# somepago/DCR

Measured on AMD Instinct MI355X. Metric: sd21_256px_finetune_imgs_per_sec, higher is better.
Workload: dtype bf16; 1 GPU; model=sd2.1-unet-865M-random-init, global_batch=16, resolution=256, seq_len=77, parallelism=dp1, optimizer=fused_adamw

## Files before the change

### dcr_amd/__main__.py

```python
import hashlib
import platform

import torch

import dcr_amd
from dcr_amd import ops


def main():
    print(f"dcr_amd {dcr_amd.__version__}")
    print(f"torch {torch.__version__} (hip {torch.version.hip})")
    print(f"python {platform.python_version()} on {platform.machine()}")
    print(f"cuda/hip device available: {torch.cuda.is_available()}")
    m = ops.ext()
    if m is None:
        print("HIP extension: NOT BUILT (run __graft_entry__.build())")
    else:
        kernels = sorted(n for n in dir(m) if not n.startswith("_"))
        from pathlib import Path
        so = Path(ops.__file__).parent / "_dcr_hip.so"
        digest = hashlib.sha256(so.read_bytes()).hexdigest()[:16]
        print(f"HIP extension: {so} (sha256 {digest})")
        print(f"  exported ops ({len(kernels)}): {', '.join(kernels)}")
    if ops.dispatch_counts:
        print(f"dispatch counts: {dict(ops.dispatch_counts)}")
    import os
    gates = ["DCR_NATIVE_CONV", "DCR_NATIVE_CONV_BWD", "DCR_NATIVE_GEMM",
             "DCR_ATTN_V4", "DCR_ATTN_BWD_V4", "DCR_HIPGRAPH",
             "DCR_ATTN_V2", "DCR_DEV_ADAMW", "DCR_PROFILE",
             "DCR_AMD_ALLOW_FALLBACK"]
    active = {g: os.environ[g] for g in gates if g in os.environ}
    desc = active if active else "defaults (native conv on; round-2 drafts off)"
    print(f"env gates: {desc}")


if __name__ == "__main__":
    main()
```

### dcr_amd/ops/hip/bindings.cpp

```cpp

#include <torch/extension.h>
#include <ATen/cuda/CUDAContext.h>

#include "dcr_launchers.h"

using namespace dcr;

namespace {

DType dtype_of(const at::Tensor& t) {
  switch (t.scalar_type()) {
    case at::kFloat: return DT_F32;
    case at::kHalf: return DT_F16;
    case at::kBFloat16: return DT_BF16;
    default: TORCH_CHECK(false, "dcr_hip: unsupported dtype ", t.scalar_type());
  }
}

hipStream_t cur_stream() {
  return at::cuda::getCurrentCUDAStream().stream();
}

at::Tensor as_f32(const at::Tensor& t) {
  return t.scalar_type() == at::kFloat ? t.contiguous()
// ... 449 lines not shown

std::vector<at::Tensor> attn_fwd_gen_lse(at::Tensor q, at::Tensor k,
                                         at::Tensor v, double scale,
                                         bool causal) {
  at::Tensor lse;
  auto o = attn_fwd_gen_impl(q, k, v, scale, causal, &lse);
  return {o, lse};
}

std::vector<at::Tensor> attn_bwd_gen(at::Tensor q, at::Tensor k, at::Tensor v,
                                     at::Tensor o, at::Tensor dO,
                                     at::Tensor lse, double scale,
                                     bool causal) {
  int64_t B, H, Lq, Lk, D;
  attn_gen_dims(q, k, v, B, H, Lq, Lk, D);
  TORCH_CHECK(k.sizes() == v.sizes(), "attn_bwd_gen: k/v shape mismatch");
  TORCH_CHECK(o.sizes() == q.sizes() && dO.sizes() == q.sizes(),
              "attn_bwd_gen: o/dO must have q's shape");
  TORCH_CHECK(o.is_cuda() && dO.is_cuda() && lse.is_cuda() &&
              o.scalar_type() == at::kBFloat16 &&
              dO.scalar_type() == at::kBFloat16 &&
              o.is_contiguous() && dO.is_contiguous(),
              "attn_bwd_gen: o/dO must be contiguous bf16 CUDA tensors");
  TORCH_CHECK(lse.scalar_type() == at::kFloat && lse.is_contiguous() &&
              lse.dim() == 2 && lse.size(0) == B * H && lse.size(1) == Lq,
              "attn_bwd_gen: lse must be contiguous fp32 [B*H, Lq]");
  auto dQ = at::empty_like(q);
  auto dK = at::empty_like(k);
  auto dV = at::empty_like(v);
  auto delta = at::empty({B * H, Lq}, q.options().dtype(at::kFloat));
  attn_bwd_gen_launch(q.data_ptr(), k.data_ptr(), v.data_ptr(), o.data_ptr(),
                      dO.data_ptr(), lse.data_ptr<float>(),
                      delta.data_ptr<float>(), dQ.data_ptr(), dK.data_ptr(),
                      dV.data_ptr(), (int)(B * H), (int)Lq, (int)Lk, (int)H,
                      (int)D, (float)scale, causal, cur_stream());
  return {dQ, dK, dV};
}

std::vector<at::Tensor> attn_fwd_v4(at::Tensor q, at::Tensor k, at::Tensor v,
                                    double scale, bool causal) {
  TORCH_CHECK(q.is_cuda() && q.scalar_type() == at::kBFloat16,
              "attn: bf16 CUDA only");
  TORCH_CHECK(q.is_contiguous() && k.is_contiguous() && v.is_contiguous());
  int64_t B, H, Lq, Lk;
  attn_dims(q, k, B, H, Lq, Lk);
  auto o = at::empty_like(q);
  auto lse = at::empty({B * H, Lq}, q.options().dtype(at::kFloat));
  attn_fwd_v4_launch(q.data_ptr(), k.data_ptr(), v.data_ptr(), o.data_ptr(),
                     lse.data_ptr<float>(), (int)(B * H), (int)Lq, (int)Lk,
                     (int)H, (float)scale, causal, cur_stream());
  return {o, lse};
}

std::vector<at::Tensor> attn_fwd_v3(at::Tensor q, at::Tensor k, at::Tensor v,
                                    double scale, bool causal) {
  TORCH_CHECK(q.is_cuda() && q.scalar_type() == at::kBFloat16,
              "attn: bf16 CUDA only");
  TORCH_CHECK(q.is_contiguous() && k.is_contiguous() && v.is_contiguous());
  int64_t B, H, Lq, Lk;
  attn_dims(q, k, B, H, Lq, Lk);
  auto o = at::empty_like(q);
  auto lse = at::empty({B * H, Lq}, q.options().dtype(at::kFloat));
  attn_fwd_v3_launch(q.data_ptr(), k.data_ptr(), v.data_ptr(), o.data_ptr(),
                     lse.data_ptr<float>(), (int)(B * H), (int)Lq, (int)Lk,
                     (int)H, (float)scale, causal, cur_stream());
  return {o, lse};
}

std::vector<at::Tensor> attn_fwd_v2(at::Tensor q, at::Tensor k, at::Tensor v,
                                    double scale, bool causal) {
  TORCH_CHECK(q.is_cuda() && q.scalar_type() == at::kBFloat16,
              "attn: bf16 CUDA only");
  TORCH_CHECK(q.is_contiguous() && k.is_contiguous() && v.is_contiguous());
  int64_t B, H, Lq, Lk;
  attn_dims(q, k, B, H, Lq, Lk);
  auto o = at::empty_like(q);
  auto lse = at::empty({B * H, Lq}, q.options().dtype(at::kFloat));
  attn_fwd_v2_launch(q.data_ptr(), k.data_ptr(), v.data_ptr(), o.data_ptr(),
                     lse.data_ptr<float>(), (int)(B * H), (int)Lq, (int)Lk,
                     (int)H, (float)scale, causal, cur_stream());
  return {o, lse};
}

std::vector<at::Tensor> attn_bwd(at::Tensor q, at::Tensor k, at::Tensor v,
                                 at::Tensor o, at::Tensor dO, at::Tensor lse,
                                 double scale, bool causal) {
  int64_t B, H, Lq, Lk;
  attn_dims(q, k, B, H, Lq, Lk);
  auto dQ = at::empty_like(q);
  auto dK = at::empty_like(k);
  auto dV = at::empty_like(v);
  auto delta = at::empty({B * H, Lq}, q.options().dtype(at::kFloat));
  attn_bwd_launch(q.data_ptr(), k.data_ptr(), v.data_ptr(), o.data_ptr(),
                  dO.contiguous().data_ptr(), lse.data_ptr<float>(),
                  delta.data_ptr<float>(), dQ.data_ptr(), dK.data_ptr(),
                  dV.data_ptr(), (int)(B * H), (int)Lq, (int)Lk, (int)H,
                  (float)scale, causal, cur_stream());
  return {dQ, dK, dV};
}

std::vector<at::Tensor> attn_bwd_v4(at::Tensor q, at::Tensor k, at::Tensor v,
                                 at::Tensor o, at::Tensor dO, at::Tensor lse,
                                 double scale, bool causal) {
  int64_t B, H, Lq, Lk;
  attn_dims(q, k, B, H, Lq, Lk);
  auto dQ = at::empty_like(q);
  auto dK = at::empty_like(k);
  auto dV = at::empty_like(v);
  auto delta = at::empty({B * H, Lq}, q.options().dtype(at::kFloat));
  attn_bwd_v4_launch(q.data_ptr(), k.data_ptr(), v.data_ptr(), o.data_ptr(),
                  dO.contiguous().data_ptr(), lse.data_ptr<float>(),
                  delta.data_ptr<float>(), dQ.data_ptr(), dK.data_ptr(),
                  dV.data_ptr(), (int)(B * H), (int)Lq, (int)Lk, (int)H,
                  (float)scale, causal, cur_stream());
  return {dQ, dK, dV};
}


at::Tensor mfma_probe(at::Tensor A, at::Tensor B) {
  TORCH_CHECK(A.is_cuda() && A.scalar_type() == at::kBFloat16);
  TORCH_CHECK(A.sizes() == at::IntArrayRef({16, 32}) &&
              B.sizes() == at::IntArrayRef({32, 16}));
  auto C = at::zeros({16, 16}, A.options().dtype(at::kFloat));
  mfma_probe_launch(A.contiguous().data_ptr(), B.contiguous().data_ptr(),
                    C.data_ptr<float>(), cur_stream());
  return C;
}

static const void* conv_bias_ptr(const c10::optional<at::Tensor>& bias,
                                 at::Tensor& keep, bool& is_bf16) {
  is_bf16 = false;
  if (!bias.has_value()) return nullptr;
  if (bias->scalar_type() == at::kBFloat16) {
    is_bf16 = true;
    keep = bias->contiguous();
  } else {
    keep = as_f32(*bias);
  }
  return keep.data_ptr();
}

at::Tensor conv2d_nhwc_fwd(at::Tensor x, at::Tensor w,
                           c10::optional<at::Tensor> bias, int64_t stride,
                           int64_t pad) {
  TORCH_CHECK(x.is_cuda() && x.scalar_type() == at::kBFloat16);
  TORCH_CHECK(x.is_contiguous(at::MemoryFormat::ChannelsLast) &&
              w.is_contiguous(at::MemoryFormat::ChannelsLast),
              "conv_nhwc: channels_last only");
  const int64_t Nb = x.size(0), C = x.size(1), Hin = x.size(2), Win = x.size(3);
  const int64_t K = w.size(0), R = w.size(2), S = w.size(3);
  TORCH_CHECK(w.size(1) == C && C % 32 == 0 && K % 64 == 0);
  TORCH_CHECK((R == 3 && S == 3) || (R == 1 && S == 1));
  const int64_t P = (Hin + 2 * pad - R) / stride + 1;
  const int64_t Q = (Win + 2 * pad - S) / stride + 1;
  auto y = at::empty({Nb, K, P, Q},
                     x.options().memory_format(at::MemoryFormat::ChannelsLast));
  at::Tensor bf;
  bool b_bf16 = false;
  const void* bp = conv_bias_ptr(bias, bf, b_bf16);
  conv_nhwc_fwd_launch(x.data_ptr(), w.data_ptr(), bp, b_bf16, y.data_ptr(), (int)Nb,
                       (int)Hin, (int)Win, (int)C, (int)K, (int)P, (int)Q,
                       (int)R, (int)S, (int)stride, (int)pad, cur_stream());
  return y;
}

static at::Tensor conv2d_nhwc_fwd_v2_impl(at::Tensor x, at::Tensor w,
                                          c10::optional<at::Tensor> bias,
                                          int64_t stride, int64_t pad,
                                          c10::optional<at::Tensor> res,
                                          c10::optional<at::Tensor> temb) {
  TORCH_CHECK(x.is_cuda() && x.scalar_type() == at::kBFloat16);
  TORCH_CHECK(x.is_contiguous(at::MemoryFormat::ChannelsLast) &&
              w.is_contiguous(at::MemoryFormat::ChannelsLast));
  const int64_t Nb = x.size(0), C = x.size(1), Hin = x.size(2), Win = x.size(3);
  const int64_t K = w.size(0), R = w.size(2), S = w.size(3);
  TORCH_CHECK(w.size(1) == C && C % 32 == 0 && K % 64 == 0);
  TORCH_CHECK((R == 3 && S == 3) || (R == 1 && S == 1));
  const int64_t P = (Hin + 2 * pad - R) / stride + 1;
  const int64_t Q = (Win + 2 * pad - S) / stride + 1;
  auto y = at::empty({Nb, K, P, Q},
                     x.options().memory_format(at::MemoryFormat::ChannelsLast));
  at::Tensor bf;
  bool b_bf16 = false;
  const void* bp = conv_bias_ptr(bias, bf, b_bf16);
  const int64_t NPQ = Nb * P * Q;
  int64_t blocks = ((NPQ + 127) / 128) * ((K + 127) / 128);
  int64_t nsteps = C * R * S / ((C % 64 == 0) ? 64 : 32);
  int splitz = 1;
  if (blocks < 384) {
    splitz = (int)std::min<int64_t>({(384 + blocks - 1) / blocks, nsteps, 16});
    if (splitz < 1) splitz = 1;
  }
  at::Tensor ws;
  float* wsp = nullptr;
  if (splitz > 1) {
    ws = at::zeros({NPQ * K}, x.options().dtype(at::kFloat));
    wsp = ws.data_ptr<float>();
  }
  const void* rp = nullptr;
  const void* tp = nullptr;
  if (res.has_value()) {
    TORCH_CHECK(res->scalar_type() == at::kBFloat16 &&
                res->is_contiguous(at::MemoryFormat::ChannelsLast) &&
                res->sizes() == y.sizes(), "conv res: NHWC bf16 same shape");
    rp = res->data_ptr();
  }
  if (temb.has_value()) {
    TORCH_CHECK(temb->scalar_type() == at::kBFloat16 &&
                temb->is_contiguous() && temb->dim() == 2 &&
                temb->size(0) == Nb && temb->size(1) == K,
                "conv temb: contiguous bf16 [N, K]");
    tp = temb->data_ptr();
  }
  conv_nhwc_fwd_v2_launch(x.data_ptr(), w.data_ptr(), bp, b_bf16, y.data_ptr(), wsp,
         splitz, rp, tp, (int)Nb, (int)Hin, (int)Win, (int)C, (int)K,
         (int)P, (int)Q, (int)R, (int)S, (int)stride,
         (int)pad, cur_stream());
  return y;
}

at::Tensor conv2d_nhwc_fwd_v2(at::Tensor x, at::Tensor w,
                              c10::optional<at::Tensor> bias, int64_t stride,
                              int64_t pad,
                              c10::optional<at::Tensor> res = c10::nullopt,
                              c10::optional<at::Tensor> temb = c10::nullopt) {
  return conv2d_nhwc_fwd_v2_impl(x, w, bias, stride, pad, res, temb);
}

std::vector<at::Tensor> conv2d_nhwc_bwd(at::Tensor dy, at::Tensor x,
                                        at::Tensor w, int64_t stride,
                                        int64_t pad) {
  TORCH_CHECK(dy.is_cuda() && dy.scalar_type() == at::kBFloat16);
  TORCH_CHECK(dy.is_contiguous(at::MemoryFormat::ChannelsLast) &&
              x.is_contiguous(at::MemoryFormat::ChannelsLast) &&
              w.is_contiguous(at::MemoryFormat::ChannelsLast));
  const int64_t Nb = x.size(0), C = x.size(1), Hin = x.size(2), Win = x.size(3);
  const int64_t K = w.size(0), R = w.size(2), S = w.size(3);
  TORCH_CHECK(C % 64 == 0 && K % 64 == 0);
  const int64_t P = dy.size(2), Q = dy.size(3);
  const int64_t NPQ = Nb * P * Q;
  int splits = (int)std::min<int64_t>(std::max<int64_t>(
      384 / std::max<int64_t>((K / 64) * (R * S * C / 32), 1), 1), 16);
  auto dw_ws = at::zeros({K * R * S * C}, x.options().dtype(at::kFloat));
  auto dW = at::empty_like(w);
  conv_bwd_weight_launch(dy.data_ptr(), x.data_ptr(), dw_ws.data_ptr<float>(),
                         (int)Nb, (int)Hin, (int)Win, (int)C, (int)K, (int)P,
                         (int)Q, (int)R, (int)S, (int)stride, (int)pad,
                         splits, dW.data_ptr(), cur_stream());
  auto dx = at::empty_like(x);
  conv_bwd_data_launch(dy.data_ptr(), w.data_ptr(), dx.data_ptr(), (int)Nb,
                       (int)Hin, (int)Win, (int)C, (int)K, (int)P, (int)Q,
                       (int)R, (int)S, (int)stride, (int)pad, cur_stream());
  auto db = at::zeros({K}, x.options().dtype(at::kFloat));
  conv_bias_grad_launch(dy.data_ptr(), db.data_ptr<float>(), NPQ, (int)K,
                        cur_stream());
  return {dx, dW, db};
}

std::vector<at::Tensor> gemm_bf16(at::Tensor A, at::Tensor B,
                                  c10::optional<at::Tensor> bias,
                                  bool ta, bool tb, bool want_dbias) {
  TORCH_CHECK(A.is_cuda() && A.scalar_type() == at::kBFloat16 &&
              B.scalar_type() == at::kBFloat16, "gemm_bf16: bf16 CUDA only");
  TORCH_CHECK(A.is_contiguous() && B.is_contiguous());
  TORCH_CHECK(A.dim() == 2 && B.dim() == 2);
  const int64_t M = ta ? A.size(1) : A.size(0);
  const int64_t K = ta ? A.size(0) : A.size(1);
  const int64_t N = tb ? B.size(1) : B.size(0);
  TORCH_CHECK((tb ? B.size(0) : B.size(1)) == K, "gemm_bf16: K mismatch");
  TORCH_CHECK(K % 8 == 0, "gemm_bf16: K % 8 != 0");
  auto C = at::empty({M, N}, A.options());
  at::Tensor bf;
  const float* bp = nullptr;
  if (bias.has_value()) {
    bf = bias->to(at::kFloat).contiguous();
    bp = bf.data_ptr<float>();
  }
  const int64_t blocks = ((M + 127) / 128) * ((N + 127) / 128);
  const int64_t nsteps = (K + 63) / 64;
  int splitz = 1;
  if (blocks < 384)
    splitz = (int)std::min<int64_t>({(384 + blocks - 1) / blocks, nsteps, 16});
  if (splitz < 1) splitz = 1;
  at::Tensor ws;
  float* wsp = nullptr;
  if (splitz > 1) {
    ws = at::zeros({M * N}, A.options().dtype(at::kFloat));
    wsp = ws.data_ptr<float>();
  }
  at::Tensor db;
  float* dbp = nullptr;
  if (want_dbias) {
    TORCH_CHECK(ta, "gemm_bf16: dbias fusion needs ta (wgrad layout)");
    db = at::zeros({M}, A.options().dtype(at::kFloat));
    dbp = db.data_ptr<float>();
  }
  gemm_bf16_launch(A.data_ptr(), B.data_ptr(), bp, C.data_ptr(), wsp, dbp,
                   M, N, (int)K, ta ? 1 : 0, tb ? 1 : 0, want_dbias ? 1 : 0,
                   splitz, cur_stream());
  if (want_dbias) return {C, db};
  return {C};
}

PYBIND11_MODULE(TORCH_EXTENSION_NAME, mod) {
  mod.def("gemm_bf16", &gemm_bf16);
  mod.def("conv2d_nhwc_bwd", &conv2d_nhwc_bwd);
  mod.def("conv2d_nhwc_fwd", &conv2d_nhwc_fwd);
  mod.def("conv2d_nhwc_fwd_v2", &conv2d_nhwc_fwd_v2,
          pybind11::arg("x"), pybind11::arg("w"), pybind11::arg("bias"),
          pybind11::arg("stride"), pybind11::arg("pad"),
          pybind11::arg("res") = c10::nullopt,
          pybind11::arg("temb") = c10::nullopt);
  mod.def("attn_fwd", &attn_fwd);
  mod.def("attn_fwd_gen", &attn_fwd_gen);
  mod.def("attn_fwd_gen_lse", &attn_fwd_gen_lse);
  mod.def("attn_bwd_gen", &attn_bwd_gen);
  mod.def("attn_fwd_v2", &attn_fwd_v2);
  mod.def("attn_fwd_v3", &attn_fwd_v3);
  mod.def("attn_fwd_v4", &attn_fwd_v4);
  mod.def("attn_bwd", &attn_bwd);
  mod.def("attn_bwd_v4", &attn_bwd_v4);
  mod.def("mfma_probe", &mfma_probe);
  mod.def("groupnorm_silu_fwd", &groupnorm_silu_fwd);
  mod.def("groupnorm_silu_bwd", &groupnorm_silu_bwd);
  mod.def("groupnorm_silu_nhwc_fwd", &groupnorm_silu_nhwc_fwd);
  mod.def("groupnorm_silu_nhwc_bwd", &groupnorm_silu_nhwc_bwd);
  mod.def("layernorm_fwd", &layernorm_fwd);
  mod.def("layernorm_bwd", &layernorm_bwd, py::arg("dy"), py::arg("x"),
          py::arg("w"), py::arg("mean"), py::arg("rstd"),
          py::arg("blocks") = 0);
  mod.def("colsum", &colsum);
  mod.def("colsum_grouped", &colsum_grouped);
  mod.def("geglu_fwd", &geglu_fwd);
  mod.def("geglu_bwd", &geglu_bwd);
  mod.def("adamw_step", &adamw_step);
  mod.def("adamw_step_bf16", &adamw_step_bf16);
  mod.def("adamw_step_dev", &adamw_step_dev);
  mod.def("adamw8_step", &adamw8_step, py::arg("p"), py::arg("g"),
          py::arg("exp_avg_q"), py::arg("exp_avg_absmax"),
          py::arg("exp_avg_sq_q"), py::arg("exp_avg_sq_absmax"), py::arg("lr"),
          py::arg("beta1"), py::arg("beta2"), py::arg("eps"), py::arg("wd"),
          py::arg("step"));
  mod.def("adamw8_step_bf16", &adamw8_step_bf16, py::arg("p"), py::arg("g"),
          py::arg("master"), py::arg("exp_avg_q"), py::arg("exp_avg_absmax"),
          py::arg("exp_avg_sq_q"), py::arg("exp_avg_sq_absmax"), py::arg("lr"),
          py::arg("beta1"), py::arg("beta2"), py::arg("eps"), py::arg("wd"),
          py::arg("step"));
  mod.def("add_noise", &add_noise);
  mod.def("get_velocity", &get_velocity);
  mod.def("cfg_combine", &cfg_combine);
  mod.def("lincomb", &lincomb);
}
```

### dcr_amd/ops/hip/dcr_launchers.h

```cpp
#pragma once

#include <hip/hip_runtime.h>

namespace dcr {

enum DType { DT_F32 = 0, DT_F16 = 1, DT_BF16 = 2 };

void gn_fwd_launch(DType dt, const void* x, const void* w, const void* b,
                   bool w_f32, void* y, float* mean, float* rstd, int NG,
                   int G, int Cg, int HW, float eps, bool silu, hipStream_t s);
void gn_bwd_launch(DType dt, const void* dy, const void* x, const void* w,
                   const void* b, bool w_f32, const float* mean,
                   const float* rstd, void* dx, float* dw, float* db, int NG,
                   int G, int Cg, int HW, bool silu, hipStream_t s);
void ln_fwd_launch(DType dt, const void* x, const void* w, const void* b,
                   bool w_f32, void* y, float* mean, float* rstd, long M,
                   int N, float eps, hipStream_t s);
void ln_bwd_launch(DType dt, const void* dy, const void* x, const void* w,
                   bool w_f32, const float* mean, const float* rstd, void* dx,
                   float* dw, float* db, long M, int N, hipStream_t s);
int ln_bwd_v2_blocks(long M, int N);
void ln_bwd_v2_launch(DType dt, const void* dy, const void* x, const void* w,
                      bool w_f32, const float* mean, const float* rstd,
                      void* dx, float* slab, void* dwdb, int blocks, long M,
                      int N, hipStream_t s);

int gn_nhwc_chunks(int N, int R);
void gn_nhwc_fwd_launch(DType dt, const void* x, const void* w, const void* b,
                        bool w_f32, void* y, float* ws, float* mean, float* rstd,
                        int N, int R, int C, int G, float eps, bool silu,
                        hipStream_t s);
void gn_nhwc_bwd_launch(DType dt, const void* dy, const void* x, const void* w,
                        const void* b, bool w_f32, const float* mean,
                        const float* rstd, float* ws, void* dx, void* dwdb,
                        int N, int R, int C, int G, bool silu,
                        hipStream_t s);

int colsum_chunks(int dt, long groups, long rows_per_group, int C, int cap);
void colsum_launch(DType dt, const void* x, float* slab, void* out_n, void* out,
                   long groups, long rows_per_group, int C, int chunks,
                   hipStream_t s);

void geglu_fwd_launch(DType dt, const void* x, void* y, long M, long N,
                      hipStream_t s);
void geglu_bwd_launch(DType dt, const void* dy, const void* x, void* dx,
                      long M, long N, hipStream_t s);
void adamw_launch(float* p, const float* g, float* m, float* v, long n,
                  float lr, float b1, float b2, float eps, float wd, long step,
                  hipStream_t s);
void adamw_bf16_launch(void* p, const void* g, float* master, float* m,
                       float* v, long n, float lr, float b1, float b2,
                       float eps, float wd, long step, hipStream_t s);
void adamw_dev_launch(int bf16, void* p, const void* g, float* master,
                      float* m, float* v, long n, float b1, float b2,
                      float eps, float wd, float max_norm, float* hyper,
                      hipStream_t s);
void adamw8_launch(int bf16, void* p, const void* g, float* master,
                   unsigned char* mq, float* mabs, unsigned char* rq,
                   float* rabs, long n, double lr, double b1, double b2,
                   double eps, double wd, long step, hipStream_t s);
void sched_launch(DType dt, int mode, const void* x0, const void* noise,
                  const float* ac, const long* t, void* out, long per_sample,
                  long total, hipStream_t s);
void cfg_launch(DType dt, const void* eu, const void* et, void* out, float s_,
                long total, hipStream_t s);
void lincomb_launch(DType dt, const void* X, const void* Y, const void* Z,
                    void* out, float a, float b, float c, long total,
                    hipStream_t s);

void attn_fwd_launch(const void* q, const void* k, const void* v, void* o,
                     float* lse, int BH, int Lq, int Lk, int H, float scale,
                     bool causal, hipStream_t s);
void attn_fwd_v2_launch(const void* q, const void* k, const void* v, void* o,
                        float* lse, int BH, int Lq, int Lk, int H, float scale,
                        bool causal, hipStream_t s);
void attn_fwd_v3_launch(const void* q, const void* k, const void* v, void* o,
                        float* lse, int BH, int Lq, int Lk, int H, float scale,
                        bool causal, hipStream_t s);
void attn_fwd_v4_launch(const void* q, const void* k, const void* v, void* o,
                        float* lse, int BH, int Lq, int Lk, int H, float scale,
                        bool causal, hipStream_t s);
void attn_fwd_gen_launch(const void* q, const void* k, const void* v, void* o,
                         float* lse, int BH, int Lq, int Lk, int H, int D,
                         float scale, bool causal, hipStream_t s);
void attn_bwd_gen_launch(const void* q, const void* k, const void* v,
                         const void* o, const void* dO, const float* lse,
                         float* delta, void* dQ, void* dK, void* dV, int BH,
                         int Lq, int Lk, int H, int D, float scale,
                         bool causal, hipStream_t s);
void attn_bwd_launch(const void* q, const void* k, const void* v,
                     const void* o, const void* dO, const float* lse,
                     float* delta, void* dQ, void* dK, void* dV, int BH,
                     int Lq, int Lk, int H, float scale, bool causal,
                     hipStream_t s);
void attn_bwd_v4_launch(const void* q, const void* k, const void* v,
                        const void* o, const void* dO, const float* lse,
                        float* delta, void* dQ, void* dK, void* dV, int BH,
                        int Lq, int Lk, int H, float scale, bool causal,
                        hipStream_t s);
void mfma_probe_launch(const void* A, const void* B, float* C, hipStream_t s);

void conv_nhwc_fwd_launch(const void* x, const void* w, const void* bias,
                          bool bias_bf16, void* y, int Nb, int Hin, int Win, int C, int K,
                          int P, int Q, int R, int S, int stride, int pad,
                          hipStream_t st);
void conv_nhwc_fwd_v2_launch(const void* x, const void* w, const void* bias,
                             bool bias_bf16, void* y, float* ws, int splitz, const void* res,
                             const void* temb, int Nb, int Hin, int Win, int C,
                             int K, int P, int Q, int R, int S, int stride,
                             int pad, hipStream_t st);
void conv_bwd_weight_launch(const void* dy, const void* x, float* dw_ws,
                            int Nb, int Hin, int Win, int C, int K, int P,
                            int Q, int R, int S, int stride, int pad,
                            int splits, void* dW_out, hipStream_t st);
void conv_bwd_data_launch(const void* dy, const void* w, void* dx, int Nb,
                          int Hin, int Win, int C, int K, int P, int Q, int R,
                          int S, int stride, int pad, hipStream_t st);
void conv_bias_grad_launch(const void* dy, float* db, long NPQ, int K,
                           hipStream_t st);

void gemm_bf16_launch(const void* A, const void* B, const float* bias,
                      void* C, float* ws, float* dbias, long M, long N, int K,
                      int ta, int tb, int want_dbias, int splitz,
                      hipStream_t st);

}
```

### dcr_amd/ops/hip/gemm.hip

```cpp

#include "dcr_common.h"

namespace dcr_gemm {

typedef __attribute__((ext_vector_type(8))) short bf16x8;
typedef __attribute__((ext_vector_type(4))) float f32x4_t;

using bf16_t = __hip_bfloat16;

template <int BK, bool T, bool COLSUM>
struct Stager {
  static constexpr int NCH = BK / 16;
  const bf16_t* __restrict__ src;
  long ld;
  long row0;
  long rows;
  int K;
  int tid;
  float colsum;

  __device__ void init(const bf16_t* s, long ld_, long row0_, long rows_,
                       int K_, int tid_) {
    src = s; ld = ld_; row0 = row0_; rows = rows_; K = K_; tid = tid_;
    colsum = 0.f;
  }
  __device__ int st_row() const { return T ? (tid & 127) : (tid >> 1); }
  __device__ int st_k() const {
    return T ? ((tid >> 7) * (BK / 2)) : ((tid & 1) * (BK / 2));
  }

  __device__ void load(int k0, uint4 (&v)[NCH]) {
#pragma unroll
    for (int t = 0; t < NCH; ++t) v[t] = make_uint4(0, 0, 0, 0);
    const long r = row0 + st_row();
    const int kb = k0 + st_k();
    if (r >= rows) return;
    if (!T) {
      const bf16_t* p = src + r * ld + kb;
      if (kb + BK / 2 <= K) {
#pragma unroll
        for (int t = 0; t < NCH; ++t)
          v[t] = reinterpret_cast<const uint4*>(p)[t];
      } else {
#pragma unroll
        for (int t = 0; t < NCH; ++t)
          if (kb + t * 8 + 8 <= K) v[t] = reinterpret_cast<const uint4*>(p)[t];
          else if (kb + t * 8 < K) {
            ushort tmp[8] = {0, 0, 0, 0, 0, 0, 0, 0};
            for (int e = 0; e < 8 && kb + t * 8 + e < K; ++e)
              tmp[e] = reinterpret_cast<const ushort*>(p)[t * 8 + e];
            v[t] = *reinterpret_cast<const uint4*>(tmp);
          }
      }
    } else {
      ushort tmp[BK / 2];
      const bf16_t* p = src + (long)kb * ld + r;
#pragma unroll
      for (int j = 0; j < BK / 2; ++j) {
        tmp[j] = (kb + j < K) ? reinterpret_cast<const ushort*>(p)[(long)j * ld]
                              : (ushort)0;
      }
      if (COLSUM) {
#pragma unroll
        for (int j = 0; j < BK / 2; ++j) {
          __hip_bfloat16 h = *reinterpret_cast<__hip_bfloat16*>(&tmp[j]);
          colsum += __bfloat162float(h);
        }
      }
#pragma unroll
      for (int t = 0; t < NCH; ++t)
        v[t] = *reinterpret_cast<const uint4*>(&tmp[t * 8]);
    }
  }

  template <int PITCH>
  __device__ void store(short* lds, const uint4 (&v)[NCH]) {
    uint4* d = reinterpret_cast<uint4*>(lds + st_row() * PITCH + st_k());
#pragma unroll
    for (int t = 0; t < NCH; ++t) d[t] = v[t];
  }
};

template <int BK, bool TA, bool TB, bool DBIAS>
__global__ __launch_bounds__(256)
void gemm_bf16_kernel(const bf16_t* __restrict__ A, const bf16_t* __restrict__ B,
                      const float* __restrict__ bias, bf16_t* __restrict__ C,
                      float* __restrict__ ws, float* __restrict__ dbias,
                      long M, long N, int K, int splitz) {
  constexpr int PITCH = BK + 8;
  __shared__ short sA[2][128 * PITCH];
  __shared__ short sB[2][128 * PITCH];

  const long m0 = (long)blockIdx.x * 128;
  const long n0 = (long)blockIdx.y * 128;

  const int lane = threadIdx.x & 63;
  const int wid = threadIdx.x >> 6;
  const int l16 = lane & 15;
  const int kgrp = lane >> 4;
  const int wr = (wid >> 1) * 64;
  const int wc = (wid & 1) * 64;

  f32x4_t acc[4][4];
#pragma unroll
  for (int i = 0; i < 4; ++i)
#pragma unroll
    for (int j = 0; j < 4; ++j) acc[i][j] = {0.f, 0.f, 0.f, 0.f};

  Stager<BK, TA, DBIAS> stA;
  Stager<BK, TB, false> stB;
  stA.init(A, TA ? M : (long)K, m0, M, K, (int)threadIdx.x);
  stB.init(B, TB ? N : (long)K, n0, N, K, (int)threadIdx.x);

  const int nsteps = (K + BK - 1) / BK;
  const int spz = (nsteps + splitz - 1) / splitz;
  const int step0 = blockIdx.z * spz;
  const int step1 = min(nsteps, step0 + spz);
  constexpr int NCH = BK / 16;

  uint4 av[NCH], bv[NCH];
  if (step0 < step1) {
    stA.load(step0 * BK, av);
    stB.load(step0 * BK, bv);
    stA.template store<PITCH>(sA[0], av);
    stB.template store<PITCH>(sB[0], bv);
  }
  __syncthreads();

  int cur = 0;
  for (int step = step0; step < step1; ++step) {
    const bool more = (step + 1 < step1);
    if (more) {
      stA.load((step + 1) * BK, av);
      stB.load((step + 1) * BK, bv);
    }

#pragma unroll
    for (int kk = 0; kk < BK / 32; ++kk) {
      bf16x8 af[4], bf[4];
#pragma unroll
      for (int i = 0; i < 4; ++i)
        af[i] = *reinterpret_cast<const bf16x8*>(
            sA[cur] + (wr + i * 16 + l16) * PITCH + kk * 32 + kgrp * 8);
#pragma unroll
      for (int j = 0; j < 4; ++j)
        bf[j] = *reinterpret_cast<const bf16x8*>(
            sB[cur] + (wc + j * 16 + l16) * PITCH + kk * 32 + kgrp * 8);
#pragma unroll
      for (int i = 0; i < 4; ++i)
#pragma unroll
        for (int j = 0; j < 4; ++j)
          acc[i][j] = __builtin_amdgcn_mfma_f32_16x16x32_bf16(af[i], bf[j],
                                                              acc[i][j], 0, 0, 0);
    }

    if (more) {
      stA.template store<PITCH>(sA[cur ^ 1], av);
      stB.template store<PITCH>(sB[cur ^ 1], bv);
      __syncthreads();
      cur ^= 1;
    }
  }

  if (DBIAS && blockIdx.y == 0) {
    const long r = m0 + stA.st_row();
    if (r < M && stA.colsum != 0.f) atomicAdd(&dbias[r], stA.colsum);
  }

#pragma unroll
  for (int i = 0; i < 4; ++i) {
#pragma unroll
    for (int rr = 0; rr < 4; ++rr) {
      const long m = m0 + wr + i * 16 + kgrp * 4 + rr;
      if (m >= M) continue;
#pragma unroll
      for (int j = 0; j < 4; ++j) {
        const long n = n0 + wc + j * 16 + l16;
        if (n >= N) continue;
        if (splitz > 1) {
          atomicAdd(&ws[m * N + n], acc[i][j][rr]);
        } else {
          float v = acc[i][j][rr] + (bias ? bias[n] : 0.f);
          C[m * N + n] = __float2bfloat16(v);
        }
      }
    }
  }
}

__global__ void gemm_finalize_kernel(const float* __restrict__ ws,
                                     const float* __restrict__ bias,
                                     bf16_t* __restrict__ y, long total,
                                     long N) {
  for (long i = (long)blockIdx.x * blockDim.x + threadIdx.x; i < total;
       i += (long)gridDim.x * blockDim.x) {
    float v = ws[i] + (bias ? bias[i % N] : 0.f);
    y[i] = __float2bfloat16(v);
  }
}

}

#include "dcr_launchers.h"

namespace dcr {

void gemm_bf16_launch(const void* A, const void* B, const float* bias,
                      void* C, float* ws, float* dbias, long M, long N, int K,
                      int ta, int tb, int want_dbias, int splitz,
                      hipStream_t st) {
  dim3 grid((unsigned)((M + 127) / 128), (unsigned)((N + 127) / 128),
            (unsigned)splitz),
      block(256);
  const auto* a = (const dcr_gemm::bf16_t*)A;
  const auto* b = (const dcr_gemm::bf16_t*)B;
  auto* c = (dcr_gemm::bf16_t*)C;

#define DCR_GEMM_LAUNCH(BK, TA, TB, DB)                                        \
  hipLaunchKernelGGL((dcr_gemm::gemm_bf16_kernel<BK, TA, TB, DB>), grid,       \
                     block, 0, st, a, b, bias, c, ws, dbias, M, N, K, splitz)

  const bool bk64 = (K % 64 == 0) || (K > 256);
  if (!ta && !tb) {
    if (bk64) DCR_GEMM_LAUNCH(64, false, false, false);
    else      DCR_GEMM_LAUNCH(32, false, false, false);
  } else if (!ta && tb) {
    if (bk64) DCR_GEMM_LAUNCH(64, false, true, false);
    else      DCR_GEMM_LAUNCH(32, false, true, false);
  } else if (ta && tb && want_dbias) {
    if (bk64) DCR_GEMM_LAUNCH(64, true, true, true);
    else      DCR_GEMM_LAUNCH(32, true, true, true);
  } else {
    if (bk64) DCR_GEMM_LAUNCH(64, true, true, false);
    else      DCR_GEMM_LAUNCH(32, true, true, false);
  }
#undef DCR_GEMM_LAUNCH

  if (splitz > 1) {
    long total = M * N;
    long blk = (total / 4 + 255) / 256;
    if (blk > 8192) blk = 8192;
    hipLaunchKernelGGL(dcr_gemm::gemm_finalize_kernel, dim3((unsigned)blk),
                       dim3(256), 0, st, ws, bias, c, total, N);
  }
}

}
```

### dcr_amd/ops/linear.py

```python
from __future__ import annotations

import os
from typing import Optional

import torch
import torch.nn.functional as F
from torch import nn

from . import use_hip, require_hip, count_dispatch


def _mode() -> str:
    return os.environ.get("DCR_NATIVE_GEMM", "0")


def _wgrad_eligible(x2d: torch.Tensor, weight: torch.Tensor) -> bool:
    M, K = x2d.shape
    N = weight.shape[0]
    return (x2d.dtype == torch.bfloat16 and weight.dtype == torch.bfloat16
            and K % 8 == 0 and N % 8 == 0 and M % 8 == 0 and M >= 4096)


def _bias_grad_enabled() -> bool:
    return os.environ.get("DCR_NATIVE_BIAS_GRAD", "1") != "0"


_BIAS_GRAD_MIN_ROWS = 64


class _BiasGradLinear(torch.autograd.Function):

    @staticmethod
    def forward(ctx, x, weight, bias):
        y = F.linear(x, weight, bias)
        ctx.save_for_backward(x, weight)
        return y

    @staticmethod
    def backward(ctx, dy):
        x, weight = ctx.saved_tensors
        dy2 = dy.reshape(-1, dy.shape[-1])
        dx = dw = db = None
        if ctx.needs_input_grad[0]:
            dx = (dy2 @ weight).view(x.shape)
        if ctx.needs_input_grad[1]:
            dw = dy2.t() @ x.reshape(-1, x.shape[-1])
        if ctx.needs_input_grad[2]:
            m = require_hip("colsum")
            count_dispatch("bias_grad")
            db = m.colsum(dy2.contiguous())
        return dx, dw, db


class _HybridLinear(torch.autograd.Function):

    @staticmethod
    def forward(ctx, x2d, weight, bias):
        y = F.linear(x2d, weight, bias)
        ctx.save_for_backward(x2d, weight)
        ctx.has_bias = bias is not None
        return y

    @staticmethod
    def backward(ctx, dy):
        x2d, weight = ctx.saved_tensors
        dy = dy.contiguous()
        dx = dy @ weight if ctx.needs_input_grad[0] else None
        dw = db = None
        if ctx.needs_input_grad[1]:
            m = require_hip("gemm_bf16")
            count_dispatch("gemm_wgrad")
            want_db = ctx.has_bias and ctx.needs_input_grad[2]
            if want_db:
                dw, db = m.gemm_bf16(dy, x2d, None, True, True, True)
                db = db.to(dy.dtype)
            else:
                (dw,) = m.gemm_bf16(dy, x2d, None, True, True, False)
        elif ctx.has_bias and ctx.needs_input_grad[2]:
            db = dy.sum(0)
        return dx, dw, db


class _FullNativeLinear(torch.autograd.Function):

    @staticmethod
    def forward(ctx, x2d, weight, bias):
        m = require_hip("gemm_bf16")
        count_dispatch("gemm")
        (y,) = m.gemm_bf16(x2d, weight, bias, False, False, False)
        ctx.save_for_backward(x2d, weight)
        ctx.has_bias = bias is not None
        return y

    @staticmethod
    def backward(ctx, dy):
        x2d, weight = ctx.saved_tensors
        m = require_hip("gemm_bf16")
        dy = dy.contiguous()
        dx = None
        if ctx.needs_input_grad[0]:
            (dx,) = m.gemm_bf16(dy, weight, None, False, True, False)
        dw = db = None
        if ctx.needs_input_grad[1]:
            if ctx.has_bias and ctx.needs_input_grad[2]:
                dw, db = m.gemm_bf16(dy, x2d, None, True, True, True)
                db = db.to(dy.dtype)
            else:
                (dw,) = m.gemm_bf16(dy, x2d, None, True, True, False)
        return dx, dw, db


def dcr_linear(x: torch.Tensor, weight: torch.Tensor,
               bias: Optional[torch.Tensor] = None) -> torch.Tensor:
    mode = _mode()
    if mode != "0" and use_hip(x) and torch.is_grad_enabled() \
            and weight.requires_grad:
        x2d = x.reshape(-1, x.shape[-1])
        if _wgrad_eligible(x2d, weight):
            fn = _FullNativeLinear if mode == "full" else _HybridLinear
            y = fn.apply(x2d.contiguous(), weight.contiguous(), bias)
            return y.reshape(*x.shape[:-1], weight.shape[0])
    if bias is not None and bias.requires_grad and use_hip(x) \
            and torch.is_grad_enabled() and _bias_grad_enabled() \
            and not torch.is_autocast_enabled() \
            and x.dtype == weight.dtype == bias.dtype \
            and x.dtype in (torch.bfloat16, torch.float16, torch.float32) \
            and x.numel() // x.shape[-1] >= _BIAS_GRAD_MIN_ROWS:
        return _BiasGradLinear.apply(x, weight, bias)
    return F.linear(x, weight, bias)


class DcrLinear(nn.Linear):

    def forward(self, x: torch.Tensor) -> torch.Tensor:
        return dcr_linear(x, self.weight, self.bias)
```

Baseline: 245.3 imgs/sec.

## Add split-K MFMA weight-gradient kernel with fused bias-grad for linear backward

```diff
diff --git a/dcr_amd/__main__.py b/dcr_amd/__main__.py
--- a/dcr_amd/__main__.py
+++ b/dcr_amd/__main__.py
@@ -26,7 +26,7 @@
         print(f"dispatch counts: {dict(ops.dispatch_counts)}")
     import os
     gates = ["DCR_NATIVE_CONV", "DCR_NATIVE_CONV_BWD", "DCR_NATIVE_GEMM",
-             "DCR_ATTN_V4", "DCR_ATTN_BWD_V4", "DCR_HIPGRAPH",
+             "DCR_NATIVE_WGRAD", "DCR_NATIVE_BIAS_GRAD", "DCR_ATTN_V4", "DCR_ATTN_BWD_V4", "DCR_HIPGRAPH",
              "DCR_ATTN_V2", "DCR_DEV_ADAMW", "DCR_PROFILE",
              "DCR_AMD_ALLOW_FALLBACK"]
     active = {g: os.environ[g] for g in gates if g in os.environ}
diff --git a/dcr_amd/ops/hip/bindings.cpp b/dcr_amd/ops/hip/bindings.cpp
--- a/dcr_amd/ops/hip/bindings.cpp
+++ b/dcr_amd/ops/hip/bindings.cpp
@@ -775,8 +775,39 @@
   return {C};
 }
 
+std::vector<at::Tensor> linear_wgrad(at::Tensor dy, at::Tensor x, bool want_db,
+                                     int64_t split, int64_t tile) {
+  TORCH_CHECK(dy.is_cuda() && x.is_cuda() &&
+              dy.scalar_type() == at::kBFloat16 &&
+              x.scalar_type() == at::kBFloat16, "linear_wgrad: bf16 CUDA only");
+  TORCH_CHECK(dy.dim() == 2 && x.dim() == 2 && dy.is_contiguous() &&
+              x.is_contiguous(), "linear_wgrad: contiguous 2-D expected");
+  const int64_t M = dy.size(0), N = dy.size(1), K = x.size(1);
+  TORCH_CHECK(x.size(0) == M, "linear_wgrad: row mismatch");
+  TORCH_CHECK(M >= 1 && N % 8 == 0 && K % 8 == 0 && N >= 8 && K >= 8,
+              "linear_wgrad: N % 8 == 0 and K % 8 == 0 expected");
+  TORCH_CHECK(N * K + N < (1LL << 31) && split >= 0 && split < (1 << 16));
+  TORCH_CHECK(M * std::max(N, K) < (1LL << 30),
+              "linear_wgrad: operands of 2 GiB and more are not supported "
+              "(32-bit buffer offsets)");
+  int tn, sp, cps;
+  linear_wgrad_plan(M, (int)N, (int)K, (int)tile, (int)split, &tn, &sp, &cps);
+  const int64_t ld = N * K + (want_db ? N : 0);
+  auto slab = at::empty({sp * ld}, dy.options().dtype(at::kFloat));
+  auto out = at::empty({ld}, dy.options());
+  linear_wgrad_launch(dy.data_ptr(), x.data_ptr(), slab.data_ptr<float>(),
+                      out.data_ptr(), M, (int)N, (int)K, want_db ? 1 : 0, tn,
+                      sp, cps, cur_stream());
+  auto dw = out.narrow(0, 0, N * K).view({N, K});
+  if (want_db) return {dw, out.narrow(0, N * K, N)};
+  return {dw};
+}
+
 PYBIND11_MODULE(TORCH_EXTENSION_NAME, mod) {
   mod.def("gemm_bf16", &gemm_bf16);
+  mod.def("linear_wgrad", &linear_wgrad, pybind11::arg("dy2d"),
+          pybind11::arg("x2d"), pybind11::arg("want_db"),
+          pybind11::arg("split") = 0, pybind11::arg("tile") = 0);
   mod.def("conv2d_nhwc_bwd", &conv2d_nhwc_bwd);
   mod.def("conv2d_nhwc_fwd", &conv2d_nhwc_fwd);
   mod.def("conv2d_nhwc_fwd_v2", &conv2d_nhwc_fwd_v2,
diff --git a/dcr_amd/ops/hip/dcr_launchers.h b/dcr_amd/ops/hip/dcr_launchers.h
--- a/dcr_amd/ops/hip/dcr_launchers.h
+++ b/dcr_amd/ops/hip/dcr_launchers.h
@@ -123,5 +123,11 @@
                       void* C, float* ws, float* dbias, long M, long N, int K,
                       int ta, int tb, int want_dbias, int splitz,
                       hipStream_t st);
+void linear_wgrad_plan(long M, int N, int K, int tile_req, int split_req,
+                       int* tile, int* split, int* chunks_per_slice);
+void linear_wgrad_launch(const void* dy, const void* x, float* slab,
+                         void* dwdb, long M, int N, int K, int want_db,
+                         int tile, int split, int chunks_per_slice,
+                         hipStream_t st);
 
 }
diff --git a/dcr_amd/ops/hip/gemm.hip b/dcr_amd/ops/hip/gemm.hip
--- a/dcr_amd/ops/hip/gemm.hip
+++ b/dcr_amd/ops/hip/gemm.hip
@@ -199,9 +199,200 @@
   }
 }
 
+
+constexpr int WG_BM = 128;
+constexpr int WG_TK = 64;
+
+typedef __attribute__((ext_vector_type(4))) short s16x4;
+typedef __attribute__((ext_vector_type(4))) unsigned u32x4;
+
+template <int T>
+__device__ __forceinline__ int wg_swz(int row) {
+  if (T == 64) return ((row >> 1) & 1) | (((row >> 3) & 1) << 1);
+  return (row & 3) | (((row >> 3) & 1) << 2);
+}
+
+template <int T>
+__device__ __forceinline__ int wg_off(int row, int col) {
+  return row * (T * 2) + ((((col >> 4) ^ wg_swz<T>(row))) << 5) + (col & 15) * 2;
+}
+
+__device__ __forceinline__ __amdgpu_buffer_rsrc_t wg_rsrc(const bf16_t* p,
+                                                          long bytes) {
+  return __builtin_amdgcn_make_buffer_rsrc(const_cast<bf16_t*>(p), 0, (int)bytes,
+                                           0x00020000);
+}
+
+template <int T>
+__device__ __forceinline__ void wg_load(__amdgpu_buffer_rsrc_t src, long ld,
+                                        long m0, bool live, int col0, int cols,
+                                        int tid, uint4 (&v)[T / 16]) {
+  constexpr int CPR = T / 8;
+  const int col = col0 + (tid % CPR) * 8;
+  const unsigned off0 =
+      live ? (unsigned)((m0 + tid / CPR) * ld + (col < cols ? col : 0)) * 2u
+           : 0x80000000u;
+#pragma unroll
+  for (int t = 0; t < T / 16; ++t) {
+    const unsigned off = off0 + (unsigned)(t * (256 / CPR) * ld) * 2u;
+    const u32x4 g = __builtin_amdgcn_raw_buffer_load_b128(src, (int)off, 0, 0);
+    v[t] = make_uint4(g.x, g.y, g.z, g.w);
+  }
+}
+
+template <int T>
+__device__ __forceinline__ void wg_store(char* img, int tid,
+                                         const uint4 (&v)[T / 16]) {
+  constexpr int CPR = T / 8;
+#pragma unroll
+  for (int t = 0; t < T / 16; ++t) {
+    const int row = tid / CPR + t * (256 / CPR);
+    *reinterpret_cast<uint4*>(img + wg_off<T>(row, (tid % CPR) * 8)) = v[t];
+  }
+}
+
+__device__ __forceinline__ void wg_colsum(const uint4& v, float (&cs)[8]) {
+  const unsigned w[4] = {v.x, v.y, v.z, v.w};
+#pragma unroll
+  for (int e = 0; e < 4; ++e) {
+    cs[2 * e] += __uint_as_float(w[e] << 16);
+    cs[2 * e + 1] += __uint_as_float(w[e] & 0xffff0000u);
+  }
+}
+
+template <int T>
+__device__ __forceinline__ bf16x8 wg_frag(const char* img, int r32, int c16,
+                                          int lane) {
+  const int row = r32 + (lane >> 4) * 8 + ((lane & 15) >> 2);
+  const int col = c16 + (lane & 3) * 4;
+  typedef __attribute__((address_space(3))) s16x4 lds_s16x4;
+  const s16x4 lo = __builtin_amdgcn_ds_read_tr16_b64_v4i16(
+      (lds_s16x4*)(img + wg_off<T>(row, col)));
+  const s16x4 hi = __builtin_amdgcn_ds_read_tr16_b64_v4i16(
+      (lds_s16x4*)(img + wg_off<T>(row + 4, col)));
+  return __builtin_shufflevector(lo, hi, 0, 1, 2, 3, 4, 5, 6, 7);
+}
+
+template <int TN, bool DB>
+__global__ __launch_bounds__(256, TN == 64 ? 2 : 1)
+void linear_wgrad_kernel(const bf16_t* __restrict__ dy,
+                         const bf16_t* __restrict__ x, float* __restrict__ slab,
+                         long M, int N, int K, int chunks_per_slice,
+                         long slab_ld, int tiles_n, int tiles_k) {
+  constexpr int NI = TN / 16, NJ = WG_TK / 16;
+  constexpr int A_BYTES = WG_BM * TN * 2, B_BYTES = WG_BM * WG_TK * 2;
+  constexpr int STAGE = A_BYTES + B_BYTES;
+  constexpr int RED_BYTES = 4 * 16 * WG_TK * 4;
+  static_assert(STAGE >= RED_BYTES, "reduction reuses the staging LDS");
+  static_assert(STAGE >= (256 / (TN / 8)) * TN * 4, "db reduction too");
+  __shared__ __attribute__((aligned(16))) char smem[STAGE];
+
+  const int tid = threadIdx.x;
+  const int lane = tid & 63;
+  const int wid = tid >> 6;
+  const int nwg = gridDim.x, ntile = tiles_n * tiles_k;
+  const int xcd = blockIdx.x % 8, q = nwg / 8, r = nwg % 8;
+  const int wg = (xcd < r ? xcd * (q + 1) : r * (q + 1) + (xcd - r) * q) +
+                 blockIdx.x / 8;
+  const int bz = wg / ntile, bt = wg % ntile;
+  const int bx = bt % tiles_n, by = bt / tiles_n;
+  const int n0 = bx * TN;
+  const int k0 = by * WG_TK;
+  const long nchunks = (M + WG_BM - 1) / WG_BM;
+  const long c0 = (long)bz * chunks_per_slice;
+  const long c1 = min(nchunks, c0 + chunks_per_slice);
+  const bool do_db = DB && by == 0;
+
+  f32x4_t acc[NI][NJ];
+#pragma unroll
+  for (int i = 0; i < NI; ++i)
+#pragma unroll
+    for (int j = 0; j < NJ; ++j) acc[i][j] = {0.f, 0.f, 0.f, 0.f};
+  float cs[8] = {0.f, 0.f, 0.f, 0.f, 0.f, 0.f, 0.f, 0.f};
+
+  char* sa = smem;
+  char* sb = smem + A_BYTES;
+  uint4 av0[TN / 16], bv0[WG_TK / 16], av1[TN / 16], bv1[WG_TK / 16];
+  const __amdgpu_buffer_rsrc_t rdy = wg_rsrc(dy, M * N * 2);
+  const __amdgpu_buffer_rsrc_t rx = wg_rsrc(x, M * K * 2);
+  auto fetch = [&](long c, uint4 (&a)[TN / 16], uint4 (&b)[WG_TK / 16]) {
+    wg_load<TN>(rdy, N, c * WG_BM, c < c1, n0, N, tid, a);
+    wg_load<WG_TK>(rx, K, c * WG_BM, c < c1, k0, K, tid, b);
+  };
+  auto step = [&](long c, uint4 (&a)[TN / 16], uint4 (&b)[WG_TK / 16]) {
+    wg_store<TN>(sa, tid, a);
+    wg_store<WG_TK>(sb, tid, b);
+    if (do_db) {
+#pragma unroll
+      for (int t = 0; t < TN / 16; ++t) wg_colsum(a[t], cs);
+    }
+    __syncthreads();
+    fetch(c + 2, a, b);
+    bf16x8 af[NI], bf[NJ];
+#pragma unroll
+    for (int i = 0; i < NI; ++i) af[i] = wg_frag<TN>(sa, wid * 32, i * 16, lane);
+#pragma unroll
+    for (int j = 0; j < NJ; ++j) bf[j] = wg_frag<WG_TK>(sb, wid * 32, j * 16, lane);
+#pragma unroll
+    for (int i = 0; i < NI; ++i)
+#pragma unroll
+      for (int j = 0; j < NJ; ++j)
+        acc[i][j] = __builtin_amdgcn_mfma_f32_16x16x32_bf16(af[i], bf[j],
+                                                            acc[i][j], 0, 0, 0);
+    __syncthreads();
+  };
+  fetch(c0, av0, bv0);
+  fetch(c0 + 1, av1, bv1);
+  for (long c = c0; c < c1; c += 2) {
+    step(c, av0, bv0);
+    step(c + 1, av1, bv1);
+  }
+
+  float* srow = slab + (long)bz * slab_ld;
+
+  float* red = reinterpret_cast<float*>(smem);
+#pragma unroll
+  for (int i = 0; i < NI; ++i) {
+    __syncthreads();
+#pragma unroll
+    for (int j = 0; j < NJ; ++j)
+#pragma unroll
+      for (int r = 0; r < 4; ++r)
+        red[(wid * 16 + (lane >> 4) * 4 + r) * WG_TK + j * 16 + (lane & 15)] =
+            acc[i][j][r];
+    __syncthreads();
+    const int rn = tid >> 4, ck = (tid & 15) * 4;
+    float4 s = *reinterpret_cast<const float4*>(red + rn * WG_TK + ck);
+#pragma unroll
+    for (int w = 1; w < 4; ++w) {
+      const float4 p =
+          *reinterpret_cast<const float4*>(red + (w * 16 + rn) * WG_TK + ck);
+      s.x += p.x; s.y += p.y; s.z += p.z; s.w += p.w;
+    }
+    const int n = n0 + i * 16 + rn, k = k0 + ck;
+    if (n < N && k < K)
+      *reinterpret_cast<float4*>(srow + (long)n * K + k) = s;
+  }
+
+  if (do_db) {
+    constexpr int CPR = TN / 8, RT = 256 / CPR;
+    __syncthreads();
+#pragma unroll
+    for (int e = 0; e < 8; ++e)
+      red[(tid / CPR) * TN + (tid % CPR) * 8 + e] = cs[e];
+    __syncthreads();
+    if (tid < TN && n0 + tid < N) {
+      float s = red[tid];
+      for (int r = 1; r < RT; ++r) s += red[r * TN + tid];
+      srow[(long)N * K + n0 + tid] = s;
+    }
+  }
+}
+
 }
 
 #include "dcr_launchers.h"
+#include "dcr_reduce.h"
 
 namespace dcr {
 
@@ -245,4 +436,50 @@
   }
 }
 
-}
+#define WG_TARGET 400
+void linear_wgrad_plan(long M, int N, int K, int tile_req, int split_req,
+                       int* tile, int* split, int* chunks_per_slice) {
+  const long nchunks = (M + dcr_gemm::WG_BM - 1) / dcr_gemm::WG_BM;
+  const long kt = (K + dcr_gemm::WG_TK - 1) / dcr_gemm::WG_TK;
+  const int tn = tile_req == 128 ? 128 : 64;
+  const long tiles = ((N + tn - 1) / tn) * kt;
+  long sp = split_req;
+  if (sp <= 0) {
+    sp = (WG_TARGET + tiles / 2) / tiles;
+    const long cap = (M * ((long)N + K)) / ((long)N * K);
+    if (sp > cap) sp = cap;
+  }
+  if (sp > nchunks) sp = nchunks;
+  if (sp < 1) sp = 1;
+  long cps = (nchunks + sp - 1) / sp;
+  if (split_req <= 0 && cps > 1) cps += cps & 1;
+  *tile = tn;
+  *chunks_per_slice = (int)cps;
+  *split = (int)((nchunks + cps - 1) / cps);
+}
+
+void linear_wgrad_launch(const void* dy, const void* x, float* slab,
+                         void* dwdb, long M, int N, int K, int want_db,
+                         int tile, int split, int chunks_per_slice,
+                         hipStream_t st) {
+  const long ld = (long)N * K + (want_db ? N : 0);
+  const int tn = (N + tile - 1) / tile;
+  const int tk = (K + dcr_gemm::WG_TK - 1) / dcr_gemm::WG_TK;
+  dim3 grid((unsigned)((long)tn * tk * split)), block(256);
+  const auto* a = (const dcr_gemm::bf16_t*)dy;
+  const auto* b = (const dcr_gemm::bf16_t*)x;
+#define DCR_WGRAD_LAUNCH(TN, DB)                                               \
+  hipLaunchKernelGGL((dcr_gemm::linear_wgrad_kernel<TN, DB>), grid, block, 0,  \
+                     st, a, b, slab, M, N, K, chunks_per_slice, ld, tn, tk)
+  if (tile == 128) {
+    if (want_db) DCR_WGRAD_LAUNCH(128, true);
+    else         DCR_WGRAD_LAUNCH(128, false);
+  } else {
+    if (want_db) DCR_WGRAD_LAUNCH(64, true);
+    else         DCR_WGRAD_LAUNCH(64, false);
+  }
+#undef DCR_WGRAD_LAUNCH
+  slab_colsum_launch<__hip_bfloat16>(slab, dwdb, split, (int)ld, ld, st);
+}
+
+}
diff --git a/dcr_amd/ops/linear.py b/dcr_amd/ops/linear.py
--- a/dcr_amd/ops/linear.py
+++ b/dcr_amd/ops/linear.py
@@ -28,12 +28,30 @@
 _BIAS_GRAD_MIN_ROWS = 64
 
 
-class _BiasGradLinear(torch.autograd.Function):
+def _native_wgrad_enabled() -> bool:
+    return os.environ.get("DCR_NATIVE_WGRAD", "1") != "0"
+
+
+_WGRAD_SMALL_TILES, _WGRAD_SMALL_MIN_ROWS = 100, 1024
+_WGRAD_MAX_TILES, _WGRAD_MIN_ROWS = 256, 8192
+
+
+def _native_wgrad_rule(M: int, N: int, K: int) -> bool:
+    if N % 8 or K % 8 or M * max(N, K) >= 1 << 30:
+        return False
+    tiles = ((N + 63) // 64) * ((K + 63) // 64)
+    if tiles <= _WGRAD_SMALL_TILES:
+        return M >= _WGRAD_SMALL_MIN_ROWS
+    return tiles <= _WGRAD_MAX_TILES and M >= _WGRAD_MIN_ROWS
+
+
+class _DefaultLinear(torch.autograd.Function):
 
     @staticmethod
-    def forward(ctx, x, weight, bias):
+    def forward(ctx, x, weight, bias, native_wgrad):
         y = F.linear(x, weight, bias)
         ctx.save_for_backward(x, weight)
+        ctx.native_wgrad = native_wgrad
         return y
 
     @staticmethod
@@ -43,13 +61,23 @@
         dx = dw = db = None
         if ctx.needs_input_grad[0]:
             dx = (dy2 @ weight).view(x.shape)
+        if ctx.native_wgrad and ctx.needs_input_grad[1]:
+            m = require_hip("linear_wgrad")
+            count_dispatch("linear_wgrad")
+            out = m.linear_wgrad(dy2.contiguous(),
+                                 x.reshape(-1, x.shape[-1]).contiguous(),
+                                 bool(ctx.needs_input_grad[2]))
+            dw = out[0]
+            if ctx.needs_input_grad[2]:
+                db = out[1]
+            return dx, dw, db, None
         if ctx.needs_input_grad[1]:
             dw = dy2.t() @ x.reshape(-1, x.shape[-1])
         if ctx.needs_input_grad[2]:
             m = require_hip("colsum")
             count_dispatch("bias_grad")
             db = m.colsum(dy2.contiguous())
-        return dx, dw, db
+        return dx, dw, db, None
 
 
 class _HybridLinear(torch.autograd.Function):
@@ -120,13 +148,19 @@
             fn = _FullNativeLinear if mode == "full" else _HybridLinear
             y = fn.apply(x2d.contiguous(), weight.contiguous(), bias)
             return y.reshape(*x.shape[:-1], weight.shape[0])
-    if bias is not None and bias.requires_grad and use_hip(x) \
-            and torch.is_grad_enabled() and _bias_grad_enabled() \
-            and not torch.is_autocast_enabled() \
-            and x.dtype == weight.dtype == bias.dtype \
-            and x.dtype in (torch.bfloat16, torch.float16, torch.float32) \
-            and x.numel() // x.shape[-1] >= _BIAS_GRAD_MIN_ROWS:
-        return _BiasGradLinear.apply(x, weight, bias)
+    if use_hip(x) and torch.is_grad_enabled() \
+            and not torch.is_autocast_enabled():
+        rows = x.numel() // x.shape[-1]
+        if weight.requires_grad and _native_wgrad_enabled() \
+                and x.dtype == weight.dtype == torch.bfloat16 \
+                and (bias is None or bias.dtype == torch.bfloat16) \
+                and _native_wgrad_rule(rows, weight.shape[0], weight.shape[1]):
+            return _DefaultLinear.apply(x, weight, bias, True)
+        if bias is not None and bias.requires_grad and _bias_grad_enabled() \
+                and x.dtype == weight.dtype == bias.dtype \
+                and x.dtype in (torch.bfloat16, torch.float16, torch.float32) \
+                and rows >= _BIAS_GRAD_MIN_ROWS:
+            return _DefaultLinear.apply(x, weight, bias, False)
     return F.linear(x, weight, bias)
 
 
```

Measured after the change: 264.0 imgs/sec (median of 6 runs). 7.6% higher.
